# proger/haloop

Measured on AMD Instinct MI355X. Metric: utterances/sec, LSTM-CTC training step (fwd + CTC loss + bwd + clip + AdamW), higher is better.
Workload: dtype bf16 (dense operands rounded to bf16, 1 MFMA per product, fp32 accumulate; fp32 state, CTC, optimizer and master weights); 1 GPU; LC-2x1024: conv(80->128,k5,s4) + 2-layer LSTM H=1024 + Linear(1024->32) + CTC, 80 frames x 80 mels, vocab 32, targets 5-10 symbols, dropout 0.2; batch_per_gpu=64, global_batch=64, frames=80, mels=80, parallelism=dp1, hip_graph=False, math=bf16

## Files before the change

### haloop_amd/csrc/lstm.hip

```cpp
#include <stdlib.h>
#include <string.h>
#include "halo_common.h"
#include "halo_internal.h"
#include "tiled_image.h"
#include "lstm_persist.h"

namespace {

enum YMode { Y_NONE = 0, Y_PLAIN = 1, Y_RELU = 2, Y_DROPOUT = 3 };

typedef __bf16 bf16x8 __attribute__((ext_vector_type(8)));

template <bool X3>
struct Packed {
    static constexpr int KB = X3 ? 32 : 16;
    static constexpr int BLOCK_BYTES = X3 ? 2048 : 1024;
    __device__ static __forceinline__ void store(void *img, int tile, int nk, int i, int k, float v) {
        const int blk = k / KB, kk = k % KB;
        char *base = (char *)img + ((long)tile * (nk / KB) + blk) * BLOCK_BYTES;
        if (X3) {
            const int lane = (kk >> 3) * 16 + i, e = kk & 7;
            const __bf16 hi = (__bf16)v;
            const __bf16 lo = (__bf16)(v - (float)hi);
            reinterpret_cast<__bf16 *>(base)[lane * 8 + e] = hi;
// ... 447 lines not shown
__device__ __forceinline__ void image_jobs_block(const ImageJobs &a, int b, float *tile) {
    int j = 0;
#pragma unroll
    for (int i = 1; i < 4; ++i)
        if (i < a.n && b >= a.job[i].first) j = i;
    const int local = b - a.job[j].first, kt = local % a.job[j].KT, rt = local / a.job[j].KT;
    if (a.job[j].tr)
        halo_img::prep_transposed_block(a.job[j].src, a.job[j].R, a.job[j].K, a.job[j].ld, a.job[j].img, a.job[j].KT, a.with_lo, kt, rt,
                                        reinterpret_cast<float (*)[halo_img::TR + 1]>(tile));
    else
        halo_img::prep_rowmajor_block(a.job[j].src, a.job[j].R, a.job[j].K, a.job[j].ld, a.job[j].img, a.job[j].KT, a.with_lo, kt, rt);
}
inline void image_jobs_add(ImageJobs &a, const float *src, int R, int K, int ld, int tr, char *img) {
    const int KT = (K + 31) / 32;
    a.job[a.n++] = {src, R, K, ld, KT, tr, a.blocks, img};
    a.blocks += ((R + 127) / 128) * KT;
}

struct Prologue2Args {
    const float *w[3]; void *wdst[3]; long w_units; int wK;
    const float *h0[2]; void *hp0[2]; float *h_rm[2]; const float *c0[2]; float *c_rm[2]; long s_units;
    unsigned *zero; long zero_units;
    unsigned *zero2; long zero2_units;
    int H, B;
    ImageJobs img;
};
template <int WMODE>
__global__ __launch_bounds__(256) void persist2_prologue_kernel(const Prologue2Args a) {
    if ((int)blockIdx.x < a.img.blocks) {
        __shared__ float tile[32 * (halo_img::TR + 1)];
        image_jobs_block(a.img, blockIdx.x, tile);
        return;
    }
    const long nw = 3 * a.w_units, ns = 2 * a.s_units;
    const long total = nw + ns + a.zero_units + a.zero2_units;
    for (long u = (blockIdx.x - a.img.blocks) * 256L + threadIdx.x; u < total; u += (long)(gridDim.x - a.img.blocks) * 256) {
        if (u < nw) {
            const int m = (int)(u / a.w_units);
            pack_unit<true, WMODE, true>(u - m * a.w_units, a.w[m], a.wdst[m], a.H, a.B, a.wK, nullptr, nullptr, nullptr);
        } else if (u < nw + ns) {
            const int l = (int)((u - nw) / a.s_units);
            pack_unit<true, 2, true>(u - nw - l * a.s_units, a.h0[l], a.hp0[l], a.H, a.B, a.H, a.h_rm[l], a.c0[l], a.c_rm[l]);
        } else if (u < nw + ns + a.zero_units) {
            reinterpret_cast<uint4 *>(a.zero)[u - nw - ns] = make_uint4(0u, 0u, 0u, 0u);
        } else {
            reinterpret_cast<uint4 *>(a.zero2)[u - nw - ns - a.zero_units] = make_uint4(0u, 0u, 0u, 0u);
        }
    }
}

struct PackPairArgs {
    const float *w[3];
    char *fwd[3], *tr[3];
    int H;
    int tile_blocks;
    Prologue2Args rest;
    char *zbase[2];
    long zstride, zunits;
    int zcount;
};
__global__ __launch_bounds__(256) void persist2_pack_pair_kernel(const PackPairArgs a) {
    __shared__ float tile[4][32][33];
    const int wave = threadIdx.x >> 6, lane = threadIdx.x & 63;
    if ((int)blockIdx.x >= a.tile_blocks && (int)blockIdx.x < a.tile_blocks + a.rest.img.blocks) {
        image_jobs_block(a.rest.img, blockIdx.x - a.tile_blocks, &tile[0][0][0]);
        return;
    }
    if ((int)blockIdx.x >= a.tile_blocks) {
        const Prologue2Args &r = a.rest;
        const long ns = 2 * r.s_units, nz = 2L * a.zcount * a.zunits, total = ns + r.zero_units + r.zero2_units + nz;
        const int first = a.tile_blocks + a.rest.img.blocks;
        for (long u = (blockIdx.x - first) * 256L + threadIdx.x; u < total; u += (long)(gridDim.x - first) * 256) {
            if (u >= ns + r.zero_units + r.zero2_units) {
                const long v = u - (ns + r.zero_units + r.zero2_units);
                const long per = (long)a.zcount * a.zunits;
                const int which = (int)(v / per);
                const long w = v % per;
                reinterpret_cast<uint4 *>(a.zbase[which] + (w / a.zunits) * a.zstride)[w % a.zunits] = make_uint4(0u, 0u, 0u, 0u);
            } else if (u < ns) {
                const int l = (int)(u / r.s_units);
                pack_unit<true, 2, true>(u - l * r.s_units, r.h0[l], r.hp0[l], r.H, r.B, r.H, r.h_rm[l], r.c0[l], r.c_rm[l]);
            } else if (u < ns + r.zero_units) {
                reinterpret_cast<uint4 *>(r.zero)[u - ns] = make_uint4(0u, 0u, 0u, 0u);
            } else {
                reinterpret_cast<uint4 *>(r.zero2)[u - ns - r.zero_units] = make_uint4(0u, 0u, 0u, 0u);
            }
        }
        return;
    }
    const int H = a.H, nkb = H / 32, nkb4 = 4 * H / 32;
    const int tiles_c = H / 32, tiles_per = (4 * H / 32) * tiles_c;
    const long t = (long)blockIdx.x * 4 + wave;
    const int m = (int)(t / tiles_per), tt = (int)(t % tiles_per);
    const int R0 = (tt / tiles_c) * 32, C0 = (tt % tiles_c) * 32;
    const float *w = a.w[m];
    const int i = lane & 15, kg = lane >> 4;
// ... 648 lines not shown
    w_ih += lo; w_hh += lo; b_ih += lo; b_hh += lo;
    if (h0) h0 += (size_t)lo * BH;
    if (c0) c0 += (size_t)lo * BH;
    HaloCtx &ctx = halo_ctx_cur();
    const bool images_by_pack = in_dim >= 64;
    if (in_dim < 64) {
        HALO_TRY(halo_gemm_f32(1, 1, T * B, 4 * H, in_dim, in, in_dim, w_ih[0], in_dim, l0.gates, 4 * H, b_ih[0], b_hh[0], 0, 0.f, 0, 0, 0,
                               nullptr, (halo_stream_t)st));
    }
    float *wp0 = reserve, *wp1 = fused_wpk(extra, hi, H), *wpi = wp1 + (size_t)4 * H * H;
    unsigned *flags = (unsigned *)((char *)reserve + reserve_flags_offset(T, B, in0, H, L));
    Prologue2Args pa;
    pa.img.n = 0; pa.img.blocks = 0; pa.img.with_lo = halo_math_mode() != HALO_MATH_BF16;
    pa.w[0] = w_hh[0]; pa.wdst[0] = wp0; pa.w[1] = w_hh[1]; pa.wdst[1] = wp1; pa.w[2] = w_ih[1]; pa.wdst[2] = wpi;
    pa.w_units = (long)(H / 16) * 4 * (H / 32) * 64; pa.wK = H;
    for (int l = 0; l < 2; ++l) {
        const LayerBufs lb = l ? l1 : l0;
        pa.h0[l] = h0 ? h0 + (size_t)l * BH : nullptr; pa.hp0[l] = lb.hp; pa.h_rm[l] = lb.h;
        pa.c0[l] = c0 ? c0 + (size_t)l * BH : nullptr; pa.c_rm[l] = lb.c;
    }
    pa.s_units = (long)((B + 15) / 16) * (H / 32) * 64;
    pa.zero = flags; pa.zero_units = (long)(PERSIST_FLAG_BYTES / 16);
    pa.zero2 = nullptr; pa.zero2_units = 0;
    pa.H = H; pa.B = B;
    ctx.packT_reserve = nullptr;
    ctx.emitT_reserve = nullptr;
    char *emit_hT0 = nullptr, *emit_hT1 = nullptr, *emit_xT1 = nullptr;
    if (ctx.lstm_expect_backward && H % 32 == 0) {
        float *wT = (float *)((char *)reserve + reserve_flags_offset(T, B, in0, H, L) + PERSIST_FLAG_BYTES);
        PackPairArgs pp;
        for (int m = 0; m < 3; ++m) { pp.w[m] = pa.w[m]; pp.fwd[m] = (char *)pa.wdst[m]; pp.tr[m] = (char *)(wT + (size_t)m * 4 * H * H); }
        pp.H = H;
        pp.tile_blocks = 3 * (4 * H / 32) * (H / 32) / 4;
        pp.rest = pa; pp.rest.w_units = 0;
        pp.rest.zero2 = reserve_bwd_flags(reserve, T, B, in0, H, L); pp.rest.zero2_units = (long)(PERSIST_FLAG_BYTES / 16);
        pp.zbase[0] = pp.zbase[1] = nullptr; pp.zstride = 0; pp.zunits = 0; pp.zcount = 0;
        ctx.emitT_reserve = nullptr;
        const bool emitT = persist_emit_enabled() && !h0 && B % 32 == 0 && H % 128 == 0 && T * B >= 32;
        if (emitT) {
            char *imgs = reserve_p2_images(reserve, T, B, in0, H, L);
            const size_t hb = halo_tiled_image_bytes(H, T * B), ib = halo_tiled_image_bytes(in0 > H ? in0 : H, T * B);
            emit_hT0 = imgs; emit_hT1 = imgs + hb + ib; emit_xT1 = emit_hT1 + hb;
            const long KT = (T * B + 31) / 32;
            pp.zbase[0] = emit_hT0; pp.zbase[1] = emit_hT1;
            pp.zstride = KT * 16384; pp.zunits = (long)(B / 32) * 16384 / 16; pp.zcount = H / 128;
            ctx.emitT_reserve = reserve;
        }
        ctx.fwdT_reserve = nullptr;
        if (images_by_pack) {
            ImageJobs &ij = pp.rest.img;
            image_jobs_add(ij, in, T * B, in_dim, in_dim, 0, img_in);
            image_jobs_add(ij, w_ih[0], 4 * H, in_dim, in_dim, 0, img_w);
            if (emitT) {
                image_jobs_add(ij, in, in_dim, T * B, in_dim, 1, emit_hT0 + halo_tiled_image_bytes(H, T * B));
                image_jobs_add(ij, w_ih[0], in_dim, 4 * H, in_dim, 1, reserve_p2_wT(reserve, T, B, in0, H, L));
                ctx.fwdT_reserve = reserve; ctx.fwdT_src[0] = in; ctx.fwdT_src[1] = w_ih[0];
            }
        }
        const unsigned rest_blocks = pack_grid((size_t)(2 * pa.s_units + pa.zero_units + pp.rest.zero2_units + 2L * pp.zcount * pp.zunits));
        hipLaunchKernelGGL(persist2_pack_pair_kernel, dim3((unsigned)(pp.tile_blocks + pp.rest.img.blocks) + rest_blocks), dim3(256), 0, st, pp);
        HALO_TRY(halo_launch_status());
        if (images_by_pack)
            HALO_TRY(halo_gemm_bf16x3_tiled(img_in, img_w, T * B, 4 * H, in_dim, l0.gates, 4 * H, b_ih[0], b_hh[0], 0, nullptr, st));
        ctx.packT_reserve = reserve;
        ctx.bwdflags_reserve = reserve;
        for (int m = 0; m < 3; ++m) ctx.packT_w[m] = pa.w[m];
    } else {
        const int dims[5] = {T, B, in0, H, L};
        const bool keep = ctx.lstm_weights_stamp != 0 && lo == 0 && ctx.packF_stamp == ctx.lstm_weights_stamp && ctx.packF_reserve == reserve &&
                          ctx.packF_w[0] == pa.w[0] && ctx.packF_w[1] == pa.w[1] && ctx.packF_w[2] == pa.w[2] &&
                          !memcmp(ctx.packF_dims, dims, sizeof(dims));
        if (keep) pa.w_units = 0;
        if (images_by_pack) {
            image_jobs_add(pa.img, in, T * B, in_dim, in_dim, 0, img_in);
            image_jobs_add(pa.img, w_ih[0], 4 * H, in_dim, in_dim, 0, img_w);
        }
        hipLaunchKernelGGL(persist2_prologue_kernel<0>, dim3((unsigned)pa.img.blocks + pack_grid((size_t)(3 * pa.w_units + 2 * pa.s_units + pa.zero_units))),
                           dim3(256), 0, st, pa);
        HALO_TRY(halo_launch_status());
        if (images_by_pack)
            HALO_TRY(halo_gemm_bf16x3_tiled(img_in, img_w, T * B, 4 * H, in_dim, l0.gates, 4 * H, b_ih[0], b_hh[0], 0, nullptr, st));
        ctx.packF_stamp = lo == 0 ? ctx.lstm_weights_stamp : 0;
        ctx.packF_reserve = reserve;
        for (int m = 0; m < 3; ++m) ctx.packF_w[m] = pa.w[m];
        memcpy(ctx.packF_dims, dims, sizeof(dims));
    }
    Persist2Fwd a;
    a.wp0 = (const char *)wp0; a.wp1 = (const char *)wp1; a.wpi = (const char *)wpi;
    a.hp0 = (char *)l0.hp; a.hp1 = (char *)l1.hp;
    a.xp = p_drop > 0.f ? (char *)fused_yp(extra, lo, T, B, H, L) : nullptr;
    a.gates0 = l0.gates; a.h0 = l0.h; a.c0 = l0.c;
    a.gates1 = l1.gates; a.h1 = l1.h; a.c1 = l1.c;
    a.b_ih1 = b_ih[1]; a.b_hh1 = b_hh[1];
    a.ydrop = p_drop > 0.f ? l0.ydrop : nullptr;
    a.y = y; a.y_stride_t = y_stride_t; a.y_stride_b = y_stride_b; a.y_mode = y ? (y_relu ? 2 : 1) : 0;
    a.drop = make_dropout(p_drop, seed, HALO_STREAM_LSTM_LAYER0 + (uint32_t)lo, offset, offset_dev);
    a.img_hT0 = emit_hT0; a.img_hT1 = emit_hT1; a.img_xT1 = emit_xT1;
    a.flags = flags;
    a.stamps = halo_lstm_persist_stamp_buffer();
    a.T = T; a.B = B; a.H = H;
    chain_begin(st);
    HALO_TRY(halo_lstm_persist2_fwd(a, st));
    chain_end(st, 0, 1, "lstm_persist2_fwd_kernel");
    for (int l = 0; l < 2; ++l) {
        const LayerBufs lb = l ? l1 : l0;
        if (hn) HALO_TRY(copy_d2d(hn + (size_t)(lo + l) * BH, lb.h + (size_t)T * BH, BH, st));
        if (cn) HALO_TRY(copy_d2d(cn + (size_t)(lo + l) * BH, lb.c + (size_t)T * BH, BH, st));
    }
    return HALO_OK;
}


inline size_t bwd_p2_offset(int T, int B, int in0, int H, int L) {
// ... 265 lines not shown
        float *dgp1 = (float *)(p2 + (((size_t)((B + 15) / 16) * 4 * H * sizeof(float) + 255) & ~(size_t)255));
        char *img_gT1 = (char *)(dgp1 + (size_t)T * PG);
        const bool can_emit = persist_emit_enabled() && B % 32 == 0;
        const bool emit0 = can_emit && in_lo_dim >= 64, emit1 = can_emit;
        const bool need_din = lo > 0 || dx != nullptr;
        float *din_out = lo > 0 ? din : dx;
        HaloCtx &ctx = halo_ctx_cur();
        const bool have_T = ctx.packT_reserve == reserve && ctx.packT_w[0] == w_hh[lo] && ctx.packT_w[1] == w_hh[hi] && ctx.packT_w[2] == w_ih[hi];
        const bool clean = have_T && ctx.bwdflags_reserve == reserve;
        ctx.bwdflags_reserve = nullptr;
        if (clean) flag_base = (char *)reserve_bwd_flags(reserve, T, B, in0, H, L);
        if (have_T) {
            float *wT = (float *)((char *)reserve + reserve_flags_offset(T, B, in0, H, L) + PERSIST_FLAG_BYTES);
            wpT0 = wT; wpT1 = wT + (size_t)4 * H * H; wpTi = wT + (size_t)8 * H * H;
        }
        Prologue2Args pa;
        pa.img.n = 0; pa.img.blocks = 0; pa.img.with_lo = 0;
        pa.w[0] = w_hh[lo]; pa.wdst[0] = wpT0; pa.w[1] = w_hh[hi]; pa.wdst[1] = wpT1; pa.w[2] = w_ih[hi]; pa.wdst[2] = wpTi;
        pa.w_units = have_T ? 0 : (long)(H / 16) * (4 * H / 32) * 64; pa.wK = 4 * H;
        for (int l = 0; l < 2; ++l) { pa.h0[l] = nullptr; pa.hp0[l] = nullptr; pa.h_rm[l] = nullptr; pa.c0[l] = nullptr; pa.c_rm[l] = nullptr; }
        pa.s_units = 0;
        pa.zero = (unsigned *)flag_base; pa.zero_units = (long)(PERSIST_FLAG_BYTES / 16);
        pa.zero2 = nullptr; pa.zero2_units = 0;
        if (emit0 && need_din && (T * B) % 128 != 0) {
            const long tile_bytes = (long)(4 * H / 32) * 16384;
            pa.zero2 = (unsigned *)(img_g + (long)((T * B) / 128) * tile_bytes); pa.zero2_units = tile_bytes / 16;
        }
        pa.H = H; pa.B = B;
        if (!clean) {
            hipLaunchKernelGGL(persist2_prologue_kernel<1>, dim3(pack_grid((size_t)(3 * pa.w_units + pa.zero_units + pa.zero2_units))), dim3(256), 0,
                               st, pa);
            HALO_TRY(halo_launch_status());
        }
        Persist2Bwd a;
        a.wpT0 = (const char *)wpT0; a.wpT1 = (const char *)wpT1; a.wpTi = (const char *)wpTi;
        a.dgp0 = (char *)dgp; a.dgp1 = (char *)dgp1;
        a.gates0 = l0.gates; a.gates1 = l1.gates; a.c0 = l0.c; a.c1 = l1.c;
        a.dc0 = dcarry; a.dc1 = dcarry1;
        a.dy = dy; a.dy_stride_t = y_stride_t; a.dy_stride_b = y_stride_b; a.dy_relu = y_relu;
        a.dhinit0 = dhn ? dhn + (size_t)lo * BH : nullptr; a.dcinit0 = dcn ? dcn + (size_t)lo * BH : nullptr;
        a.dhinit1 = dhn ? dhn + (size_t)hi * BH : nullptr; a.dcinit1 = dcn ? dcn + (size_t)hi * BH : nullptr;
        a.drop = make_dropout(p_drop, seed, HALO_STREAM_LSTM_LAYER0 + (uint32_t)lo, offset, offset_dev);
        a.flags = (unsigned *)flag_base;
        a.abort_word = (unsigned *)((char *)workspace + bwd_flags_offset(T, B, in0, H, L));
        a.stamps = halo_lstm_persist_stamp_buffer();
        a.img_rows0 = emit0 && need_din ? img_g : nullptr;
// ... 177 lines not shown
```

### haloop_amd/csrc/lstm_persist.h

```cpp
#pragma once
#include <hip/hip_runtime.h>
#include "halo_common.h"

constexpr int PERSIST_FLAG_HEADER = 16;
constexpr int PERSIST_MAX_BLOCKS = 256;
constexpr int PERSIST_REPLICAS = 8;
constexpr int PERSIST_REPLICA_WORDS = 1024;
constexpr size_t PERSIST_FLAG_BYTES = (size_t)PERSIST_REPLICAS * PERSIST_REPLICA_WORDS * sizeof(unsigned);

struct PersistFwd {
    const char *wp;
    char *hp;
    float *gates;
    float *h;
    float *c;
    float *y;
    long y_stride_t, y_stride_b;
    int y_mode;
    DropoutCfg drop;
    unsigned *flags;
    unsigned *status;
    int mute;
    unsigned long long *stamps;
    int poll_mode;
// ... 61 lines not shown
    float *gates0, *gates1;
    const float *c0, *c1;
    float *dc0, *dc1;
    const float *dy;
    long dy_stride_t, dy_stride_b;
    int dy_relu;
    const float *dhinit0, *dcinit0, *dhinit1, *dcinit1;
    DropoutCfg drop;
    unsigned *flags;
    unsigned *abort_word;
   
    unsigned *status;
    unsigned long long *stamps;
    char *img_rows0, *img_cols0, *img_cols1;
    float *bias_part0, *bias_part1;
    int skip_dg0, skip_dg1;
    int poll_mode, replica_shift, nap;
    int T, B, H;
    int bt0, nbt;
    unsigned epoch0;
};

bool halo_lstm_persist2_ok(int T, int B, int H, int L);
void halo_lstm_persist2_enable(int on);
void halo_lstm_interleave_enable(int on);
int halo_lstm_persist2_fwd(const Persist2Fwd &a, hipStream_t st);
int halo_lstm_persist2_bwd(const Persist2Bwd &a, hipStream_t st);
int halo_lstm_persist2x_fwd(const Persist2Fwd &a, hipStream_t st);
int halo_lstm_persist2x_bwd(const Persist2Bwd &a, hipStream_t st);
```

### haloop_amd/csrc/lstm_persist2.hip

```cpp
#include <stdlib.h>
#include "halo_common.h"
#include "halo_internal.h"
#include "lstm_persist.h"
#include "lstm_persist_dev.h"

namespace {

struct Fwd2Shared {
    float (*red)[4][4][256];
    float (*hbuf)[16][16];
    int *s_abort;
    unsigned *s_published;
};

template <int KBQ>
__device__ __forceinline__ void fwd2_layer0_waves(const Persist2Fwd &p, const Fwd2Shared sh, int jt, int bt, int wave, int lane, int u) {
    const int wq = wave & 3;
    const int H = p.H, B = p.B, T = p.T;
    const int NJ = H / 16, NBT = (B + 15) / 16, nkb = H / 32, j0 = jt * 16;
    bf16x8 wr[4][KBQ];
#pragma unroll
    for (int g = 0; g < 4; ++g)
#pragma unroll
        for (int i = 0; i < KBQ; ++i)
            wr[g][i] = *reinterpret_cast<const bf16x8 *>(p.wp0 + (((long)jt * 4 + g) * nkb + wq * KBQ + i) * 2048 + lane * 16);
    const int ci = u >> 4, cj = u & 15;
    const int b = bt * 16 + ci;
    const bool cell = b < B;
    const int BH = B * H;
    const int e0 = b * H + j0 + cj;
    float cst = 0.f, gin[4] = {0.f, 0.f, 0.f, 0.f};
    float dmul = (cell && p.xp) ? dropout_mult(p.drop, (uint64_t)e0) : 1.f;
    if (cell) {
        cst = p.c0[e0];
#pragma unroll
        for (int g = 0; g < 4; ++g) gin[g] = p.gates0[b * 4 * H + g * H + j0 + cj];
    }
    const __amdgpu_buffer_rsrc_t hp0_rsrc = make_rsrc(p.hp0), hp1_rsrc = make_rsrc(p.hp1);
    const __amdgpu_buffer_rsrc_t x_rsrc = p.xp ? make_rsrc(p.xp) : hp0_rsrc;
    const int my_replica = (xcc_id() + p.replica_shift) % PERSIST_REPLICAS;
    const int btl = bt - p.bt0;
    const unsigned *grp_flags = p.flags + my_replica * PERSIST_REPLICA_WORDS + PERSIST_FLAG_HEADER + btl * NJ;
    for (int s = 0; s <= T + 1; ++s) {
        if (wave == 0) stamp(p.stamps, T + 2, s, 0, lane);
        const bool act0 = s < T, act1 = s >= 2;
        bool ok = true;
        if (s > 0 && wave == 1) ok = poll_group(grp_flags, 0, NJ, p.epoch0 + (unsigned)s, lane, p.nap);
        if (!ok && lane == 0) {
            *sh.s_abort = 1;
            raise_abort(p.flags, p.status);
        }
        lds_barrier();
        if (*sh.s_abort) return;
        if (wave == 0) stamp(p.stamps, T + 2, s, 1, lane);
        if (act0) {
            const int img = ((s * NBT + bt) * nkb + wq * KBQ) * 2048;
            bf16x8 ah[KBQ];
#pragma unroll
            for (int i = 0; i < KBQ; ++i) ah[i] = load_sc1_u(hp0_rsrc, lane * 16, img + i * 2048);
            __builtin_amdgcn_sched_barrier(0);
            f32x4 acc[4];
#pragma unroll
            for (int g = 0; g < 4; ++g) acc[g] = f32x4{0.f, 0.f, 0.f, 0.f};
#pragma unroll
            for (int i = 0; i < KBQ; ++i)
#pragma unroll
                for (int g = 0; g < 4; ++g) acc[g] = __builtin_amdgcn_mfma_f32_16x16x32_bf16(ah[i], wr[g][i], acc[g], 0, 0, 0);
            const int r = lane & 15, q = lane >> 4;
#pragma unroll
            for (int g = 0; g < 4; ++g)
#pragma unroll
                for (int e = 0; e < 4; ++e) sh.red[0][wq][g][(4 * q + e) * 16 + r] = acc[g][e];
        }
        lds_barrier();
        if (wave == 0) stamp(p.stamps, T + 2, s, 2, lane);
        float ig = 0.f, fg = 0.f, gg = 0.f, og = 0.f, h = 0.f, xv = 0.f;
        if (act0) {
            if (cell) {
                float pre[4];
#pragma unroll
                for (int g = 0; g < 4; ++g) {
                    float sum = 0.f;
#pragma unroll
                    for (int k = 0; k < 4; ++k) sum += sh.red[0][k][g][u];
                    pre[g] = sum + gin[g];
                }
                h = persist2_fwd_cell(pre, cst, ig, fg, gg, og);
                if (p.xp) xv = h * dmul;
            }
            sh.hbuf[0][ci][cj] = h;
            if (p.xp) sh.hbuf[1][ci][cj] = xv;
        }
        lds_barrier();
        if (wave == 0) stamp(p.stamps, T + 2, s, 3, lane);
        if ((wave == 3 && act0) || (wave == 2 && act1)) {
            const int sel = lane >> 5, kg = (lane >> 4) & 1, row = lane & 15;
            const float(*src)[16] = wave == 2 ? sh.hbuf[2] : sh.hbuf[sel];
            bf16x8 hi;
#pragma unroll
            for (int e = 0; e < 8; ++e) hi[e] = (__bf16)src[row][kg * 8 + e];
            const int within = (jt >> 1) * 2048 + (((jt & 1) * 2 + kg) * 16 + row) * 16;
            if (wave == 3) {
                if (sel == 0) store_sc1(hp0_rsrc, (((s + 1) * NBT + bt) * nkb) * 2048 + within, hi);
                else if (p.xp) store_sc1(x_rsrc, ((s * NBT + bt) * nkb) * 2048 + within, hi);
            } else if (sel == 0) {
                store_sc1(hp1_rsrc, (((s - 1) * NBT + bt) * nkb) * 2048 + within, hi);
            }
            asm volatile("s_waitcnt vmcnt(0)" ::: "memory");
            unsigned old = 0;
            if (lane == 0) old = atomicAdd(sh.s_published, 1u);
            old = __builtin_amdgcn_readfirstlane(old);
            const unsigned target = (unsigned)((s + 1 < T ? s + 1 : T) + (s >= 2 ? s - 1 : 0));
            if (old + 1u == target && (int)blockIdx.x != p.mute) publish_epoch(p.flags, btl * NJ + jt, p.epoch0 + (unsigned)(s + 1), lane);
            stamp(p.stamps, T + 2, s, wave == 3 ? 4 : 5, lane);
        } else if (wave == 3 && !act0 && !act1) {
            publish_epoch(p.flags, btl * NJ + jt, p.epoch0 + (unsigned)(s + 1), lane);
        }
        if (p.img_hT0 && ((wave == 3 && act0) || (wave == 2 && act1))) {
            const int sel = lane >> 5, kg = (lane >> 4) & 1, row = lane & 15;
            const float(*src)[16] = wave == 2 ? sh.hbuf[2] : (sel == 1 && p.xp ? sh.hbuf[1] : sh.hbuf[0]);
            const int tb = wave == 2 ? s - 1 : (sel == 0 ? s + 1 : s);
            char *img = wave == 2 ? (sel == 0 ? p.img_hT1 : nullptr) : (sel == 0 ? p.img_hT0 : p.img_xT1);
            if (img && tb < T) {
                bf16x8 hit;
#pragma unroll
                for (int e = 0; e < 8; ++e) hit[e] = (__bf16)src[kg * 8 + e][row];
                const int grow = j0 + row, kcol = tb * B + bt * 16 + kg * 8;
                const int KT = (T * B + 31) >> 5;
                const long blk = ((long)(grow >> 7) * KT + (kcol >> 5)) * 2;
                const int r = grow & 127, cc = (kcol & 31) >> 3;
                *reinterpret_cast<bf16x8 *>(img + blk * 8192 + r * 64 + ((cc ^ ((r >> 2) & 3)) << 4)) = hit;
            }
        }
        if (act0 && cell) {
            float *gp = p.gates0 + (s * B + b) * 4 * H + j0 + cj;
            gp[0] = ig; gp[H] = fg; gp[2 * H] = gg; gp[3 * H] = og;
            p.c0[(s + 1) * BH + e0] = cst;
            p.h0[(s + 1) * BH + e0] = h;
            if (p.ydrop) p.ydrop[s * BH + e0] = xv;
            if (p.xp && s + 1 < T) dmul = dropout_mult(p.drop, (uint64_t)((long)(s + 1) * BH + e0));
            if (s + 1 < T) {
#pragma unroll
                for (int g = 0; g < 4; ++g) gin[g] = p.gates0[((s + 1) * B + b) * 4 * H + g * H + j0 + cj];
            }
        }
    }
}

template <int KBQ>
__device__ __forceinline__ void fwd2_layer1_waves(const Persist2Fwd &p, const Fwd2Shared sh, char *wi_lds, int jt, int bt, int wave, int lane,
                                                  int u) {
    constexpr int NWREG = KBQ >= 8 ? 2 : 0;
    constexpr int NWLDS = 4 * KBQ - NWREG;
    const int wq = wave & 3;
    const int H = p.H, B = p.B, T = p.T;
    const int NBT = (B + 15) / 16, nkb = H / 32, j0 = jt * 16;
    bf16x8 wr[4][KBQ];
#pragma unroll
    for (int g = 0; g < 4; ++g)
#pragma unroll
        for (int i = 0; i < KBQ; ++i)
            wr[g][i] = *reinterpret_cast<const bf16x8 *>(p.wp1 + (((long)jt * 4 + g) * nkb + wq * KBQ + i) * 2048 + lane * 16);
    bf16x8 wir[NWREG > 0 ? NWREG : 1];
    char *my_wi = wi_lds + (long)wq * NWLDS * 1024 + lane * 16;
#pragma unroll
    for (int i = 0; i < KBQ; ++i)
#pragma unroll
        for (int g = 0; g < 4; ++g) {
            const bf16x8 v = *reinterpret_cast<const bf16x8 *>(p.wpi + (((long)jt * 4 + g) * nkb + wq * KBQ + i) * 2048 + lane * 16);
            if (i * 4 + g < NWREG) wir[i * 4 + g < NWREG ? i * 4 + g : 0] = v;
            else *reinterpret_cast<bf16x8 *>(my_wi + (i * 4 + g - NWREG) * 1024) = v;
            if (g == 3 && (i & 3) == 3) __builtin_amdgcn_sched_barrier(0);
// ... 1 lines not shown
    const int ci = u >> 4, cj = u & 15;
    const int b = bt * 16 + ci;
    const bool cell = b < B;
    const int BH = B * H;
    const int e0 = b * H + j0 + cj;
    float cst = 0.f, bias[4] = {0.f, 0.f, 0.f, 0.f};
    if (cell) {
        cst = p.c1[e0];
#pragma unroll
        for (int g = 0; g < 4; ++g) bias[g] = p.b_ih1[g * H + j0 + cj] + p.b_hh1[g * H + j0 + cj];
    }
    const __amdgpu_buffer_rsrc_t hp1_rsrc = make_rsrc(p.hp1);
    const __amdgpu_buffer_rsrc_t x_rsrc = make_rsrc(p.xp ? p.xp : p.hp0);
    f32x4 xacc[4];
#pragma unroll
    for (int g = 0; g < 4; ++g) xacc[g] = f32x4{0.f, 0.f, 0.f, 0.f};
    for (int s = 0; s <= T + 1; ++s) {
        if (wave == 4) stamp(p.stamps, T + 2, s, 8, lane);
        const bool act1 = s >= 2, xin = s >= 1 && s <= T;
        const int t = s - 2;
        lds_barrier();
        if (*sh.s_abort) return;
        bf16x8 ax[KBQ];
        if (xin) {
            const int ximg = (((p.xp ? s - 1 : s) * NBT + bt) * nkb + wq * KBQ) * 2048;
#pragma unroll
            for (int i = 0; i < KBQ; ++i) ax[i] = load_sc1_u(x_rsrc, lane * 16, ximg + i * 2048);
        }
        if (act1) {
            const int img = ((t * NBT + bt) * nkb + wq * KBQ) * 2048;
            bf16x8 ah[KBQ];
#pragma unroll
            for (int i = 0; i < KBQ; ++i) ah[i] = load_sc1_u(hp1_rsrc, lane * 16, img + i * 2048);
            __builtin_amdgcn_sched_barrier(0);
#pragma unroll
            for (int i = 0; i < KBQ; ++i)
#pragma unroll
                for (int g = 0; g < 4; ++g) xacc[g] = __builtin_amdgcn_mfma_f32_16x16x32_bf16(ah[i], wr[g][i], xacc[g], 0, 0, 0);
            const int r = lane & 15, q = lane >> 4;
#pragma unroll
            for (int g = 0; g < 4; ++g)
#pragma unroll
                for (int e = 0; e < 4; ++e) sh.red[1][wq][g][(4 * q + e) * 16 + r] = xacc[g][e];
        }
        lds_barrier();
        float ig = 0.f, fg = 0.f, gg = 0.f, og = 0.f, h = 0.f;
        if (act1) {
            if (cell) {
                float pre[4];
#pragma unroll
                for (int g = 0; g < 4; ++g) {
                    float sum = 0.f;
#pragma unroll
                    for (int k = 0; k < 4; ++k) sum += sh.red[1][k][g][u];
                    pre[g] = sum + bias[g];
                }
                h = persist2_fwd_cell(pre, cst, ig, fg, gg, og);
            }
            sh.hbuf[2][ci][cj] = h;
        }
        lds_barrier();
        if (act1 && cell) {
            float *gp = p.gates1 + (t * B + b) * 4 * H + j0 + cj;
            gp[0] = ig; gp[H] = fg; gp[2 * H] = gg; gp[3 * H] = og;
            p.c1[(t + 1) * BH + e0] = cst;
            p.h1[(t + 1) * BH + e0] = h;
            if (p.y_mode != 0) p.y[(long)t * p.y_stride_t + (long)b * p.y_stride_b + j0 + cj] = p.y_mode == 2 ? fmaxf(h, 0.f) : h;
        }
        if (wave == 4) stamp(p.stamps, T + 2, s, 7, lane);
#pragma unroll
        for (int g = 0; g < 4; ++g) xacc[g] = f32x4{0.f, 0.f, 0.f, 0.f};
        if (xin) {
#pragma unroll
            for (int i = 0; i < KBQ; ++i) {
                bf16x8 w[4];
#pragma unroll
                for (int g = 0; g < 4; ++g)
                    w[g] = i * 4 + g < NWREG ? wir[i * 4 + g < NWREG ? i * 4 + g : 0]
                                             : *reinterpret_cast<const bf16x8 *>(my_wi + (i * 4 + g - NWREG) * 1024);
#pragma unroll
                for (int g = 0; g < 4; ++g) xacc[g] = __builtin_amdgcn_mfma_f32_16x16x32_bf16(ax[i], w[g], xacc[g], 0, 0, 0);
                if (i & 1) __builtin_amdgcn_sched_barrier(0);
            }
        }
        if (wave == 4) stamp(p.stamps, T + 2, s, 6, lane);
    }
}

template <int KBQ>
__global__ __launch_bounds__(512, 2) void lstm_persist2_fwd_kernel(const Persist2Fwd p) {
    __shared__ float red[2][4][4][256];
    __shared__ __attribute__((aligned(16))) float hbuf[3][16][16];
    __shared__ int s_abort;
    __shared__ unsigned s_published;
    extern __shared__ __attribute__((aligned(16))) char wi_lds[];
    const int tid = threadIdx.x, lane = tid & 63;
    const int wave = __builtin_amdgcn_readfirstlane(tid >> 6);
    int jt, bt;
    map_block(blockIdx.x, gridDim.x, p.H / 16, p.nbt, jt, bt);
    bt += p.bt0;
    if (tid == 0) { s_abort = 0; s_published = 0; }
    if (wave == 0) stamp(p.stamps, p.T + 2, 0, 14, lane);
    const Fwd2Shared sh = {red, hbuf, &s_abort, &s_published};
    if (wave < 4) fwd2_layer0_waves<KBQ>(p, sh, jt, bt, wave, lane, tid & 255);
    else fwd2_layer1_waves<KBQ>(p, sh, wi_lds, jt, bt, wave, lane, tid & 255);
    if (wave == 0) stamp(p.stamps, p.T + 2, 0, 15, lane);
}

struct Bwd2Shared {
    float (*red)[4][256];
    float (*dgbuf)[4][16][16];
    int *s_abort;
    unsigned *s_published;
};

struct Bwd2Cell {
    float gv[4], cc, cprev, dcarry;
    __device__ __forceinline__ void update(float dh, float (&dg)[4]) { dcarry = persist2_bwd_cell(gv, cc, cprev, dcarry, dh, dg); }
};

template <int KC>
__device__ __forceinline__ void bwd2_layer0_waves(const Persist2Bwd &p, const Bwd2Shared sh, int jt, int bt, int wave, int lane, int u) {
    constexpr int KBW = 4 * KC, CH = 4, NCH = KBW / CH, NBUF = 3;
    const int wq = wave & 3;
    const int H = p.H, B = p.B, T = p.T, K = 4 * H;
    const int NJ = H / 16, NBT = (B + 15) / 16, nkb4 = K / 32, j0 = jt * 16;
    bf16x8 wr[KBW];
#pragma unroll
// ... 318 lines not shown
}

}

void halo_lstm_persist2_enable(int on) { halo_ctx_cur().lstm_persistent2 = on ? 1 : 0; }
void halo_lstm_interleave_enable(int on) { halo_ctx_cur().lstm_interleave = on ? 1 : 0; }

bool halo_lstm_persist2_ok(int T, int B, int H, int L) {
    static const bool env_off = getenv("HALO_LSTM_PERSIST2") && atoi(getenv("HALO_LSTM_PERSIST2")) == 0;
    if (env_off || !halo_ctx_cur().lstm_persistent2) return false;
    if (!halo_lstm_persist_ok(16, H) || B <= 0 || !halo_lstm_persist_fits(T, B, H)) return false;
    if (halo_math_mode() != HALO_MATH_BF16 || L < 2) return false;
    if (H % 128 != 0 || H > 1024 || T < 1) return false;
    const long nbt = (B + 15) / 16;
    if ((long)(T + 2) * nbt * (4 * H / 32) * 2048 >= (1L << 31)) return false;
    if ((long)(T + 1) * B * 4 * H >= (1L << 31)) return false;
    return H / 16 <= cu_count2() && PERSIST_FLAG_HEADER + 2L * tiles_per_launch(H) * (H / 16) <= PERSIST_REPLICA_WORDS;
}

inline bool interleave_on() {
    static const bool env_off = getenv("HALO_LSTM_INTERLEAVE") && atoi(getenv("HALO_LSTM_INTERLEAVE")) == 0;
    return !env_off && halo_ctx_cur().lstm_interleave != 0;
}

template <typename A, typename F, typename FX>
int launch_groups(const A &a0, int steps, F launch_one, FX launch_pairs) {
    const int nbt = (a0.B + 15) / 16, per = tiles_per_launch(a0.H);
    const bool pairs = nbt > per && interleave_on() && (long)(a0.T + 1) * a0.B * 4 * a0.H * (long)sizeof(float) < (1L << 31);
    for (int bt0 = 0, g = 0; bt0 < nbt; ++g) {
        A a = a0;
        const int left = nbt - bt0;
        a.bt0 = bt0; a.epoch0 = (unsigned)g * (unsigned)(steps + 2);
        int rc;
        const int two = min(2 * per, left) & ~1;
        if (pairs && two > per) {
            a.nbt = two;
            rc = launch_pairs(a);
        } else {
            a.nbt = min(per, left);
            rc = launch_one(a, (a.H / 16) * a.nbt);
        }
        if (rc != HALO_OK) return rc;
        bt0 += a.nbt;
    }
    return HALO_OK;
}

int halo_lstm_persist2_fwd(const Persist2Fwd &a0, hipStream_t st) {
    const int kbq = a0.H / 128;
    const size_t dyn = (size_t)4 * 1024 * (4 * kbq - (kbq >= 8 ? 2 : 0));
    return launch_groups(a0, a0.T + 2, [&](const Persist2Fwd &a, int blocks) {
        switch (kbq) {
            case 2: return launch2(lstm_persist2_fwd_kernel<2>, a, blocks, dyn, st);
            case 4: return launch2(lstm_persist2_fwd_kernel<4>, a, blocks, dyn, st);
            case 6: return launch2(lstm_persist2_fwd_kernel<6>, a, blocks, dyn, st);
            case 8: return launch2(lstm_persist2_fwd_kernel<8>, a, blocks, dyn, st);
            default: return (int)HALO_ENOTSUP;
        }
    }, [&](const Persist2Fwd &a) { return halo_lstm_persist2x_fwd(a, st); });
}

int halo_lstm_persist2_bwd(const Persist2Bwd &a0, hipStream_t st) {
    const int kc = a0.H / 128;
    const size_t dyn = (size_t)4 * 4 * kc * 1024;
    return launch_groups(a0, a0.T + 1, [&](const Persist2Bwd &a, int blocks) {
        switch (kc) {
            case 2: return launch2(lstm_persist2_bwd_kernel<2>, a, blocks, dyn, st);
            case 4: return launch2(lstm_persist2_bwd_kernel<4>, a, blocks, dyn, st);
            case 6: return launch2(lstm_persist2_bwd_kernel<6>, a, blocks, dyn, st);
            case 8: return launch2(lstm_persist2_bwd_kernel<8>, a, blocks, dyn, st);
            default: return (int)HALO_ENOTSUP;
        }
    }, [&](const Persist2Bwd &a) { return halo_lstm_persist2x_bwd(a, st); });
}
```

Before: 156,400 utterances/s.

## Replace persistent LSTM forward flag polling with data-embedded sentinel flags

Prefills the next-step hidden-state and dropout input images with an all-ones sentinel in the prologue. The forward persistent kernel then spins on the data itself until no sentinel remains, replacing epoch flag publication, atomics and group polling. Stored values that happen to match the sentinel are nudged by one ulp so they are never mistaken for unwritten data. This removes a store-wait-publish-poll round trip per timestep but adds sentinel-writing traffic and a small numeric perturbation, and it relies on the loads seeing fully written 16-byte vectors.

```diff
diff --git a/haloop_amd/csrc/lstm.hip b/haloop_amd/csrc/lstm.hip
--- a/haloop_amd/csrc/lstm.hip
+++ b/haloop_amd/csrc/lstm.hip
@@ -493,9 +493,15 @@
     const float *h0[2]; void *hp0[2]; float *h_rm[2]; const float *c0[2]; float *c_rm[2]; long s_units;
     unsigned *zero; long zero_units;
     unsigned *zero2; long zero2_units;
+    char *arm[3]; int narm; long arm_units;
     int H, B;
     ImageJobs img;
 };
+__device__ __forceinline__ void arm_unit(const Prologue2Args &a, long v) {
+    const int m = (int)(v / a.arm_units);
+    const long w = v - m * a.arm_units;
+    *reinterpret_cast<uint4 *>(a.arm[m] + (w >> 6) * 2048 + (w & 63) * 16) = make_uint4(~0u, ~0u, ~0u, ~0u);
+}
 template <int WMODE>
 __global__ __launch_bounds__(256) void persist2_prologue_kernel(const Prologue2Args a) {
     if ((int)blockIdx.x < a.img.blocks) {
@@ -503,10 +509,12 @@
         image_jobs_block(a.img, blockIdx.x, tile);
         return;
     }
-    const long nw = 3 * a.w_units, ns = 2 * a.s_units;
-    const long total = nw + ns + a.zero_units + a.zero2_units;
+    const long nw = 3 * a.w_units, ns = 2 * a.s_units, na = (long)a.narm * a.arm_units;
+    const long total = nw + ns + a.zero_units + a.zero2_units + na;
     for (long u = (blockIdx.x - a.img.blocks) * 256L + threadIdx.x; u < total; u += (long)(gridDim.x - a.img.blocks) * 256) {
-        if (u < nw) {
+        if (u >= total - na) {
+            arm_unit(a, u - (total - na));
+        } else if (u < nw) {
             const int m = (int)(u / a.w_units);
             pack_unit<true, WMODE, true>(u - m * a.w_units, a.w[m], a.wdst[m], a.H, a.B, a.wK, nullptr, nullptr, nullptr);
         } else if (u < nw + ns) {
@@ -539,10 +547,13 @@
     }
     if ((int)blockIdx.x >= a.tile_blocks) {
         const Prologue2Args &r = a.rest;
-        const long ns = 2 * r.s_units, nz = 2L * a.zcount * a.zunits, total = ns + r.zero_units + r.zero2_units + nz;
+        const long ns = 2 * r.s_units, nz = 2L * a.zcount * a.zunits, na = (long)r.narm * r.arm_units;
+        const long total = ns + r.zero_units + r.zero2_units + nz + na;
         const int first = a.tile_blocks + a.rest.img.blocks;
         for (long u = (blockIdx.x - first) * 256L + threadIdx.x; u < total; u += (long)(gridDim.x - first) * 256) {
-            if (u >= ns + r.zero_units + r.zero2_units) {
+            if (u >= total - na) {
+                arm_unit(r, u - (total - na));
+            } else if (u >= ns + r.zero_units + r.zero2_units) {
                 const long v = u - (ns + r.zero_units + r.zero2_units);
                 const long per = (long)a.zcount * a.zunits;
                 const int which = (int)(v / per);
@@ -1237,6 +1248,15 @@
     pa.s_units = (long)((B + 15) / 16) * (H / 32) * 64;
     pa.zero = flags; pa.zero_units = (long)(PERSIST_FLAG_BYTES / 16);
     pa.zero2 = nullptr; pa.zero2_units = 0;
+    char *xp = p_drop > 0.f ? (char *)fused_yp(extra, lo, T, B, H, L) : nullptr;
+    pa.narm = 0; pa.arm_units = 0;
+    if (halo_lstm_persist2_fwd_armed(T, B, H)) {
+        const size_t image = (size_t)((B + 15) / 16) * (H / 32) * 2048;
+        pa.arm[pa.narm++] = (char *)l0.hp + image;
+        pa.arm[pa.narm++] = (char *)l1.hp + image;
+        if (xp) pa.arm[pa.narm++] = xp;
+        pa.arm_units = (long)T * (long)(image / 2048) * 64;
+    }
     pa.H = H; pa.B = B;
     ctx.packT_reserve = nullptr;
     ctx.emitT_reserve = nullptr;
@@ -1272,7 +1292,8 @@
                 ctx.fwdT_reserve = reserve; ctx.fwdT_src[0] = in; ctx.fwdT_src[1] = w_ih[0];
             }
         }
-        const unsigned rest_blocks = pack_grid((size_t)(2 * pa.s_units + pa.zero_units + pp.rest.zero2_units + 2L * pp.zcount * pp.zunits));
+        const unsigned rest_blocks = pack_grid((size_t)(2 * pa.s_units + pa.zero_units + pp.rest.zero2_units + 2L * pp.zcount * pp.zunits +
+                                                        (long)pa.narm * pa.arm_units));
         hipLaunchKernelGGL(persist2_pack_pair_kernel, dim3((unsigned)(pp.tile_blocks + pp.rest.img.blocks) + rest_blocks), dim3(256), 0, st, pp);
         HALO_TRY(halo_launch_status());
         if (images_by_pack)
@@ -1290,7 +1311,8 @@
             image_jobs_add(pa.img, in, T * B, in_dim, in_dim, 0, img_in);
             image_jobs_add(pa.img, w_ih[0], 4 * H, in_dim, in_dim, 0, img_w);
         }
-        hipLaunchKernelGGL(persist2_prologue_kernel<0>, dim3((unsigned)pa.img.blocks + pack_grid((size_t)(3 * pa.w_units + 2 * pa.s_units + pa.zero_units))),
+        hipLaunchKernelGGL(persist2_prologue_kernel<0>, dim3((unsigned)pa.img.blocks + pack_grid((size_t)(3 * pa.w_units + 2 * pa.s_units + pa.zero_units +
+                                                                                                      (long)pa.narm * pa.arm_units))),
                            dim3(256), 0, st, pa);
         HALO_TRY(halo_launch_status());
         if (images_by_pack)
@@ -1303,7 +1325,7 @@
     Persist2Fwd a;
     a.wp0 = (const char *)wp0; a.wp1 = (const char *)wp1; a.wpi = (const char *)wpi;
     a.hp0 = (char *)l0.hp; a.hp1 = (char *)l1.hp;
-    a.xp = p_drop > 0.f ? (char *)fused_yp(extra, lo, T, B, H, L) : nullptr;
+    a.xp = xp;
     a.gates0 = l0.gates; a.h0 = l0.h; a.c0 = l0.c;
     a.gates1 = l1.gates; a.h1 = l1.h; a.c1 = l1.c;
     a.b_ih1 = b_ih[1]; a.b_hh1 = b_hh[1];
@@ -1615,6 +1637,7 @@
         pa.s_units = 0;
         pa.zero = (unsigned *)flag_base; pa.zero_units = (long)(PERSIST_FLAG_BYTES / 16);
         pa.zero2 = nullptr; pa.zero2_units = 0;
+        pa.narm = 0; pa.arm_units = 0;
         if (emit0 && need_din && (T * B) % 128 != 0) {
             const long tile_bytes = (long)(4 * H / 32) * 16384;
             pa.zero2 = (unsigned *)(img_g + (long)((T * B) / 128) * tile_bytes); pa.zero2_units = tile_bytes / 16;
diff --git a/haloop_amd/csrc/lstm_persist.h b/haloop_amd/csrc/lstm_persist.h
--- a/haloop_amd/csrc/lstm_persist.h
+++ b/haloop_amd/csrc/lstm_persist.h
@@ -107,6 +107,8 @@
 };
 
 bool halo_lstm_persist2_ok(int T, int B, int H, int L);
+bool halo_lstm_persist2_dataflag();
+bool halo_lstm_persist2_fwd_armed(int T, int B, int H);
 void halo_lstm_persist2_enable(int on);
 void halo_lstm_interleave_enable(int on);
 int halo_lstm_persist2_fwd(const Persist2Fwd &a, hipStream_t st);
diff --git a/haloop_amd/csrc/lstm_persist2.hip b/haloop_amd/csrc/lstm_persist2.hip
--- a/haloop_amd/csrc/lstm_persist2.hip
+++ b/haloop_amd/csrc/lstm_persist2.hip
@@ -5,6 +5,31 @@
 #include "lstm_persist_dev.h"
 
 namespace {
+
+__device__ __forceinline__ bf16x8 unarm(bf16x8 v) {
+    u32x4 w = __builtin_bit_cast(u32x4, v);
+    if ((w.x & 0xffffu) == 0xffffu) w.x -= 1u;
+    return __builtin_bit_cast(bf16x8, w);
+}
+template <int N>
+__device__ __forceinline__ bool armed_lane(const bf16x8 (&f)[N]) {
+    bool a = false;
+#pragma unroll
+    for (int i = 0; i < N; ++i) a |= (__builtin_bit_cast(u32x4, f[i]).x & 0xffffu) == 0xffffu;
+    return a;
+}
+__device__ __forceinline__ bool rearm_wait(unsigned long long &t0, int pass, int nap) {
+    const unsigned long long now = __builtin_amdgcn_s_memrealtime();
+    if (pass == 0) t0 = now;
+    else if (now - t0 > SPIN_TIMEOUT_TICKS) return false;
+    if (nap == 1) __builtin_amdgcn_s_sleep(1);
+    else if (nap == 2) __builtin_amdgcn_s_sleep(4);
+    else if (nap == 3) __builtin_amdgcn_s_sleep(16);
+    return true;
+}
+__device__ __forceinline__ void stamp_value(unsigned long long *stamps, int T, int step, int point, int lane, unsigned v) {
+    if (stamps && lane == 0) stamps[((long)blockIdx.x * T + step) * 16 + point] = v;
+}
 
 struct Fwd2Shared {
     float (*red)[4][4][256];
@@ -13,7 +38,7 @@
     unsigned *s_published;
 };
 
-template <int KBQ>
+template <int KBQ, bool DF>
 __device__ __forceinline__ void fwd2_layer0_waves(const Persist2Fwd &p, const Fwd2Shared sh, int jt, int bt, int wave, int lane, int u) {
     const int wq = wave & 3;
     const int H = p.H, B = p.B, T = p.T;
@@ -44,11 +69,13 @@
     for (int s = 0; s <= T + 1; ++s) {
         if (wave == 0) stamp(p.stamps, T + 2, s, 0, lane);
         const bool act0 = s < T, act1 = s >= 2;
-        bool ok = true;
-        if (s > 0 && wave == 1) ok = poll_group(grp_flags, 0, NJ, p.epoch0 + (unsigned)s, lane, p.nap);
-        if (!ok && lane == 0) {
-            *sh.s_abort = 1;
-            raise_abort(p.flags, p.status);
+        if (!DF) {
+            bool ok = true;
+            if (s > 0 && wave == 1) ok = poll_group(grp_flags, 0, NJ, p.epoch0 + (unsigned)s, lane, p.nap);
+            if (!ok && lane == 0) {
+                *sh.s_abort = 1;
+                raise_abort(p.flags, p.status);
+            }
         }
         lds_barrier();
         if (*sh.s_abort) return;
@@ -56,16 +83,28 @@
         if (act0) {
             const int img = ((s * NBT + bt) * nkb + wq * KBQ) * 2048;
             bf16x8 ah[KBQ];
-#pragma unroll
-            for (int i = 0; i < KBQ; ++i) ah[i] = load_sc1_u(hp0_rsrc, lane * 16, img + i * 2048);
-            __builtin_amdgcn_sched_barrier(0);
             f32x4 acc[4];
-#pragma unroll
-            for (int g = 0; g < 4; ++g) acc[g] = f32x4{0.f, 0.f, 0.f, 0.f};
-#pragma unroll
-            for (int i = 0; i < KBQ; ++i)
-#pragma unroll
-                for (int g = 0; g < 4; ++g) acc[g] = __builtin_amdgcn_mfma_f32_16x16x32_bf16(ah[i], wr[g][i], acc[g], 0, 0, 0);
+            unsigned long long t0 = 0;
+            for (int pass = 0;; ++pass) {
+#pragma unroll
+                for (int i = 0; i < KBQ; ++i) ah[i] = load_sc1_u(hp0_rsrc, lane * 16, img + i * 2048);
+                __builtin_amdgcn_sched_barrier(0);
+#pragma unroll
+                for (int g = 0; g < 4; ++g) acc[g] = f32x4{0.f, 0.f, 0.f, 0.f};
+#pragma unroll
+                for (int i = 0; i < KBQ; ++i)
+#pragma unroll
+                    for (int g = 0; g < 4; ++g) acc[g] = __builtin_amdgcn_mfma_f32_16x16x32_bf16(ah[i], wr[g][i], acc[g], 0, 0, 0);
+                if (!DF) break;
+                if (!__any(armed_lane<KBQ>(ah))) {
+                    if (wave == 0) { stamp(p.stamps, T + 2, s, 10, lane); stamp_value(p.stamps, T + 2, s, 11, lane, (unsigned)pass); }
+                    break;
+                }
+                if (!rearm_wait(t0, pass, p.nap)) {
+                    if (lane == 0) { *sh.s_abort = 1; raise_abort(p.flags, p.status); }
+                    break;
+                }
+            }
             const int r = lane & 15, q = lane >> 4;
 #pragma unroll
             for (int g = 0; g < 4; ++g)
@@ -73,6 +112,7 @@
                 for (int e = 0; e < 4; ++e) sh.red[0][wq][g][(4 * q + e) * 16 + r] = acc[g][e];
         }
         lds_barrier();
+        if (DF && *sh.s_abort) return;
         if (wave == 0) stamp(p.stamps, T + 2, s, 2, lane);
         float ig = 0.f, fg = 0.f, gg = 0.f, og = 0.f, h = 0.f, xv = 0.f;
         if (act0) {
@@ -99,21 +139,27 @@
             bf16x8 hi;
 #pragma unroll
             for (int e = 0; e < 8; ++e) hi[e] = (__bf16)src[row][kg * 8 + e];
+            if (DF) hi = unarm(hi);
             const int within = (jt >> 1) * 2048 + (((jt & 1) * 2 + kg) * 16 + row) * 16;
+            const bool store = !DF || (int)blockIdx.x != p.mute;
             if (wave == 3) {
-                if (sel == 0) store_sc1(hp0_rsrc, (((s + 1) * NBT + bt) * nkb) * 2048 + within, hi);
-                else if (p.xp) store_sc1(x_rsrc, ((s * NBT + bt) * nkb) * 2048 + within, hi);
-            } else if (sel == 0) {
+                if (sel == 0 && store) store_sc1(hp0_rsrc, (((s + 1) * NBT + bt) * nkb) * 2048 + within, hi);
+                else if (sel == 1 && p.xp && store) store_sc1(x_rsrc, ((s * NBT + bt) * nkb) * 2048 + within, hi);
+            } else if (sel == 0 && store) {
                 store_sc1(hp1_rsrc, (((s - 1) * NBT + bt) * nkb) * 2048 + within, hi);
             }
-            asm volatile("s_waitcnt vmcnt(0)" ::: "memory");
-            unsigned old = 0;
-            if (lane == 0) old = atomicAdd(sh.s_published, 1u);
-            old = __builtin_amdgcn_readfirstlane(old);
-            const unsigned target = (unsigned)((s + 1 < T ? s + 1 : T) + (s >= 2 ? s - 1 : 0));
-            if (old + 1u == target && (int)blockIdx.x != p.mute) publish_epoch(p.flags, btl * NJ + jt, p.epoch0 + (unsigned)(s + 1), lane);
-            stamp(p.stamps, T + 2, s, wave == 3 ? 4 : 5, lane);
-        } else if (wave == 3 && !act0 && !act1) {
+            if (DF) {
+                stamp(p.stamps, T + 2, s, wave == 3 ? 4 : 5, lane);
+            } else {
+                asm volatile("s_waitcnt vmcnt(0)" ::: "memory");
+                unsigned old = 0;
+                if (lane == 0) old = atomicAdd(sh.s_published, 1u);
+                old = __builtin_amdgcn_readfirstlane(old);
+                const unsigned target = (unsigned)((s + 1 < T ? s + 1 : T) + (s >= 2 ? s - 1 : 0));
+                if (old + 1u == target && (int)blockIdx.x != p.mute) publish_epoch(p.flags, btl * NJ + jt, p.epoch0 + (unsigned)(s + 1), lane);
+                stamp(p.stamps, T + 2, s, wave == 3 ? 4 : 5, lane);
+            }
+        } else if (!DF && wave == 3 && !act0 && !act1) {
             publish_epoch(p.flags, btl * NJ + jt, p.epoch0 + (unsigned)(s + 1), lane);
         }
         if (p.img_hT0 && ((wave == 3 && act0) || (wave == 2 && act1))) {
@@ -147,7 +193,7 @@
     }
 }
 
-template <int KBQ>
+template <int KBQ, bool DF>
 __device__ __forceinline__ void fwd2_layer1_waves(const Persist2Fwd &p, const Fwd2Shared sh, char *wi_lds, int jt, int bt, int wave, int lane,
                                                   int u) {
     constexpr int NWREG = KBQ >= 8 ? 2 : 0;
@@ -195,28 +241,62 @@
         lds_barrier();
         if (*sh.s_abort) return;
         bf16x8 ax[KBQ];
-        if (xin) {
-            const int ximg = (((p.xp ? s - 1 : s) * NBT + bt) * nkb + wq * KBQ) * 2048;
-#pragma unroll
-            for (int i = 0; i < KBQ; ++i) ax[i] = load_sc1_u(x_rsrc, lane * 16, ximg + i * 2048);
-        }
-        if (act1) {
-            const int img = ((t * NBT + bt) * nkb + wq * KBQ) * 2048;
+        if constexpr (DF) {
+            const int ximg = ((min(max(p.xp ? s - 1 : s, 0), p.xp ? T - 1 : T) * NBT + bt) * nkb + wq * KBQ) * 2048;
+            const int img = ((max(t, 0) * NBT + bt) * nkb + wq * KBQ) * 2048;
             bf16x8 ah[KBQ];
-#pragma unroll
-            for (int i = 0; i < KBQ; ++i) ah[i] = load_sc1_u(hp1_rsrc, lane * 16, img + i * 2048);
-            __builtin_amdgcn_sched_barrier(0);
-#pragma unroll
-            for (int i = 0; i < KBQ; ++i)
-#pragma unroll
-                for (int g = 0; g < 4; ++g) xacc[g] = __builtin_amdgcn_mfma_f32_16x16x32_bf16(ah[i], wr[g][i], xacc[g], 0, 0, 0);
-            const int r = lane & 15, q = lane >> 4;
-#pragma unroll
-            for (int g = 0; g < 4; ++g)
-#pragma unroll
-                for (int e = 0; e < 4; ++e) sh.red[1][wq][g][(4 * q + e) * 16 + r] = xacc[g][e];
-        }
-        lds_barrier();
+            unsigned long long t0 = 0;
+            for (int pass = 0;; ++pass) {
+#pragma unroll
+                for (int i = 0; i < KBQ; ++i) ax[i] = load_sc1_u(x_rsrc, lane * 16, ximg + i * 2048);
+#pragma unroll
+                for (int i = 0; i < KBQ; ++i) ah[i] = load_sc1_u(hp1_rsrc, lane * 16, img + i * 2048);
+                const bool bx = armed_lane<KBQ>(ax), bh = armed_lane<KBQ>(ah);
+                if (!__any((xin && bx) || (act1 && bh))) {
+                    if (wave == 4) { stamp(p.stamps, T + 2, s, 12, lane); stamp_value(p.stamps, T + 2, s, 13, lane, (unsigned)pass); }
+                    break;
+                }
+                if (!rearm_wait(t0, pass, p.nap)) {
+                    if (lane == 0) { *sh.s_abort = 1; raise_abort(p.flags, p.status); }
+                    break;
+                }
+            }
+            if (act1) {
+#pragma unroll
+                for (int i = 0; i < KBQ; ++i)
+#pragma unroll
+                    for (int g = 0; g < 4; ++g) xacc[g] = __builtin_amdgcn_mfma_f32_16x16x32_bf16(ah[i], wr[g][i], xacc[g], 0, 0, 0);
+                const int r = lane & 15, q = lane >> 4;
+#pragma unroll
+                for (int g = 0; g < 4; ++g)
+#pragma unroll
+                    for (int e = 0; e < 4; ++e) sh.red[1][wq][g][(4 * q + e) * 16 + r] = xacc[g][e];
+            }
+        } else {
+            if (xin) {
+                const int ximg = (((p.xp ? s - 1 : s) * NBT + bt) * nkb + wq * KBQ) * 2048;
+#pragma unroll
+                for (int i = 0; i < KBQ; ++i) ax[i] = load_sc1_u(x_rsrc, lane * 16, ximg + i * 2048);
+            }
+            if (act1) {
+                const int img = ((t * NBT + bt) * nkb + wq * KBQ) * 2048;
+                bf16x8 ah[KBQ];
+#pragma unroll
+                for (int i = 0; i < KBQ; ++i) ah[i] = load_sc1_u(hp1_rsrc, lane * 16, img + i * 2048);
+                __builtin_amdgcn_sched_barrier(0);
+#pragma unroll
+                for (int i = 0; i < KBQ; ++i)
+#pragma unroll
+                    for (int g = 0; g < 4; ++g) xacc[g] = __builtin_amdgcn_mfma_f32_16x16x32_bf16(ah[i], wr[g][i], xacc[g], 0, 0, 0);
+                const int r = lane & 15, q = lane >> 4;
+#pragma unroll
+                for (int g = 0; g < 4; ++g)
+#pragma unroll
+                    for (int e = 0; e < 4; ++e) sh.red[1][wq][g][(4 * q + e) * 16 + r] = xacc[g][e];
+            }
+        }
+        lds_barrier();
+        if (DF && *sh.s_abort) return;
         float ig = 0.f, fg = 0.f, gg = 0.f, og = 0.f, h = 0.f;
         if (act1) {
             if (cell) {
@@ -260,7 +340,7 @@
     }
 }
 
-template <int KBQ>
+template <int KBQ, bool DF>
 __global__ __launch_bounds__(512, 2) void lstm_persist2_fwd_kernel(const Persist2Fwd p) {
     __shared__ float red[2][4][4][256];
     __shared__ __attribute__((aligned(16))) float hbuf[3][16][16];
@@ -275,8 +355,8 @@
     if (tid == 0) { s_abort = 0; s_published = 0; }
     if (wave == 0) stamp(p.stamps, p.T + 2, 0, 14, lane);
     const Fwd2Shared sh = {red, hbuf, &s_abort, &s_published};
-    if (wave < 4) fwd2_layer0_waves<KBQ>(p, sh, jt, bt, wave, lane, tid & 255);
-    else fwd2_layer1_waves<KBQ>(p, sh, wi_lds, jt, bt, wave, lane, tid & 255);
+    if (wave < 4) fwd2_layer0_waves<KBQ, DF>(p, sh, jt, bt, wave, lane, tid & 255);
+    else fwd2_layer1_waves<KBQ, DF>(p, sh, wi_lds, jt, bt, wave, lane, tid & 255);
     if (wave == 0) stamp(p.stamps, p.T + 2, 0, 15, lane);
 }
 
@@ -641,11 +721,20 @@
     static const bool env_off = getenv("HALO_LSTM_INTERLEAVE") && atoi(getenv("HALO_LSTM_INTERLEAVE")) == 0;
     return !env_off && halo_ctx_cur().lstm_interleave != 0;
 }
+inline bool pairs_for(int T, int B, int H) {
+    return (B + 15) / 16 > tiles_per_launch(H) && interleave_on() && (long)(T + 1) * B * 4 * H * (long)sizeof(float) < (1L << 31);
+}
+
+bool halo_lstm_persist2_dataflag() {
+    static const bool on = !(getenv("HALO_PERSIST_DATAFLAG") && atoi(getenv("HALO_PERSIST_DATAFLAG")) == 0);
+    return on;
+}
+bool halo_lstm_persist2_fwd_armed(int T, int B, int H) { return halo_lstm_persist2_dataflag() && !pairs_for(T, B, H); }
 
 template <typename A, typename F, typename FX>
 int launch_groups(const A &a0, int steps, F launch_one, FX launch_pairs) {
     const int nbt = (a0.B + 15) / 16, per = tiles_per_launch(a0.H);
-    const bool pairs = nbt > per && interleave_on() && (long)(a0.T + 1) * a0.B * 4 * a0.H * (long)sizeof(float) < (1L << 31);
+    const bool pairs = pairs_for(a0.T, a0.B, a0.H);
     for (int bt0 = 0, g = 0; bt0 < nbt; ++g) {
         A a = a0;
         const int left = nbt - bt0;
@@ -668,12 +757,17 @@
 int halo_lstm_persist2_fwd(const Persist2Fwd &a0, hipStream_t st) {
     const int kbq = a0.H / 128;
     const size_t dyn = (size_t)4 * 1024 * (4 * kbq - (kbq >= 8 ? 2 : 0));
+    const bool df = halo_lstm_persist2_fwd_armed(a0.T, a0.B, a0.H);
     return launch_groups(a0, a0.T + 2, [&](const Persist2Fwd &a, int blocks) {
-        switch (kbq) {
-            case 2: return launch2(lstm_persist2_fwd_kernel<2>, a, blocks, dyn, st);
-            case 4: return launch2(lstm_persist2_fwd_kernel<4>, a, blocks, dyn, st);
-            case 6: return launch2(lstm_persist2_fwd_kernel<6>, a, blocks, dyn, st);
-            case 8: return launch2(lstm_persist2_fwd_kernel<8>, a, blocks, dyn, st);
+        switch (kbq * 2 + (df ? 1 : 0)) {
+            case 4: return launch2(lstm_persist2_fwd_kernel<2, false>, a, blocks, dyn, st);
+            case 5: return launch2(lstm_persist2_fwd_kernel<2, true>, a, blocks, dyn, st);
+            case 8: return launch2(lstm_persist2_fwd_kernel<4, false>, a, blocks, dyn, st);
+            case 9: return launch2(lstm_persist2_fwd_kernel<4, true>, a, blocks, dyn, st);
+            case 12: return launch2(lstm_persist2_fwd_kernel<6, false>, a, blocks, dyn, st);
+            case 13: return launch2(lstm_persist2_fwd_kernel<6, true>, a, blocks, dyn, st);
+            case 16: return launch2(lstm_persist2_fwd_kernel<8, false>, a, blocks, dyn, st);
+            case 17: return launch2(lstm_persist2_fwd_kernel<8, true>, a, blocks, dyn, st);
             default: return (int)HALO_ENOTSUP;
         }
     }, [&](const Persist2Fwd &a) { return halo_lstm_persist2x_fwd(a, st); });
```

Measured after the change: 160,800 utterances/s, median of 6. 2.8% higher.
